# dalek-cryptography/zkp

Hardware: AMD Instinct MI355X
Metric: proofs/sec + batch-verifies/sec, CMZ13 10-attr credential, 1/2/4/8 MI355X (higher is better)
Workload: dtype u32x9 (29-bit limbs, u64 accumulate)

## Files before the change

include/zkp_mi355x.h:

```cpp
#ifndef ZKP_MI355X_H
#define ZKP_MI355X_H

#include <stddef.h>
#include <stdint.h>

#ifdef __cplusplus
extern "C" {
#endif

#define ZKP_OK 0
#define ZKP_ERR_HIP (-1)
#define ZKP_ERR_ARG (-2)
#define ZKP_ERR_NO_DEVICE (-3)
#define ZKP_ERR_OOM (-4)

#define ZKP_VARTIME 0
#define ZKP_CT 1

typedef struct zkp_ctx zkp_ctx;

int zkp_ctx_create(zkp_ctx** out, int device_id);
void zkp_ctx_destroy(zkp_ctx* ctx);
int zkp_ctx_set_stream(zkp_ctx* ctx, void* hip_stream);
int zkp_ctx_synchronize(zkp_ctx* ctx);
// ... 226 lines not shown
  ZKP_K_COUNT = 9
};
int zkp_ctx_last_timing(zkp_ctx* ctx, float* kernel_ms , float* total_ms);
int zkp_ctx_last_kernels(zkp_ctx* ctx, int kind, char* buf, size_t cap);
int zkp_ctx_set_profiling(zkp_ctx* ctx, int enabled);

#ifdef ZKP_BUILD_TEST_HOOKS
int zkp_debug_quad_selftest(zkp_ctx* ctx, uint32_t n, const uint8_t* pairs , uint8_t* out );
int zkp_debug_row_selftest(zkp_ctx* ctx, uint32_t n, const uint8_t* pairs , uint8_t* out );
int zkp_debug_wave_cycles(zkp_ctx* ctx, uint64_t* out, uint32_t cap);
int zkp_debug_sha512(zkp_ctx* ctx, uint64_t n, const uint8_t* msgs, const uint64_t* offsets , uint8_t* out );
int zkp_debug_last_schedule(zkp_ctx* ctx, char* buf, size_t cap);
int zkp_debug_ragged_blocks(const uint8_t* transcripts, uint32_t N, uint32_t* idx, uint32_t* blocks, uint32_t cap);
int zkp_debug_fill_workspace(zkp_ctx* ctx, size_t min_bytes, uint32_t word);
size_t zkp_debug_ws_bytes(zkp_ctx* ctx);
enum { ZKP_TESTOPT_DUMMY_LAUNCHES = 1001, ZKP_TESTOPT_GENERIC_CLASSIFIER = 1002, ZKP_TESTOPT_WAVE_CYCLES = 1003, ZKP_TESTOPT_PIP_MERGE = 1004, ZKP_TESTOPT_VOUCH_REDUCED = 1005 };
#endif

#ifdef __cplusplus
}
#endif
#endif
```

zkp_amd/csrc/comb_tables.h:

```cpp
#pragma once
#include "quad.h"
#include "stmt_pairs.h"

namespace zkp {

template <int TEETH>
struct comb_cfg {
  static_assert(TEETH == 4 || TEETH == 8 || TEETH == 16 || TEETH == 32, "teeth");
  static constexpr int BITS = 256 / TEETH;
  static constexpr int WINDOWS = BITS / 4;
  static constexpr int ENTRIES = 8 * TEETH + 1;
};
constexpr int comb_entries(int teeth) { return 8 * teeth + 1; }
constexpr int LADDER_ENTRIES = 8;

__device__ __forceinline__ void q_store_cached(dev_ext* dst, const qcached& c, int q) {
  uint32_t* w = reinterpret_cast<uint32_t*>(dst) + 9 * q;
#pragma unroll
  for (int i = 0; i < 9; ++i) w[i] = c.c.v[i];
}

__global__ void __launch_bounds__(256)
k_comb_slots(uint32_t n_points, const uint32_t* __restrict__ uses, uint32_t comb_min, uint32_t group_min, uint32_t max_tables,
             uint32_t* __restrict__ counter, uint32_t* __restrict__ slot_of, uint32_t* __restrict__ slot_pt, uint32_t* __restrict__ group_start,
// ... 274 lines not shown
        ge_cached_cmov(sel, n0, (uint32_t)(mag == 1));
        ge_cached_cmov(sel, n1, (uint32_t)(mag == 2));
#pragma unroll 1
        for (uint32_t h = 1; h < 4; ++h) {
          ge_cached c0, c1;
          load_comb_entry(c0, row + 2 * h + 0);
          load_comb_entry(c1, row + 2 * h + 1);
          ge_cached_cmov(sel, c0, (uint32_t)(mag == 2 * h + 1));
          ge_cached_cmov(sel, c1, (uint32_t)(mag == 2 * h + 2));
        }
        const dev_ext* next = (j + 1 < TEETH) ? row + 8 : tbl;
        load_comb_entry(n0, next + 0);
        load_comb_entry(n1, next + 1);
        if (fold && nidx == (int)SC_FOLD16_TOP_NIBBLE + 1) continue;
        ge_cached_cneg(sel, neg);
        if (w == cfg::WINDOWS - 1 && j == 0) ge_from_cached(acc, sel);
        else ge_add_cached(acc, acc, sel);
      }
    }
    if (fold) ge_cneg(acc, flip);
  } else {
#pragma unroll 1
    for (int w = cfg::WINDOWS - 1; w >= 0; --w) {
      if (w != cfg::WINDOWS - 1) {
        ge_double4(acc);
      }
#pragma unroll 1
      for (int j = 0; j < TEETH; ++j) {
        const int nidx = j * cfg::WINDOWS + w;
        const uint32_t nib = (ecol[256 * (nidx >> 3)] >> (4 * (nidx & 7))) & 15u;
        const uint32_t neg = (uint32_t)(nib < 8u);
        const uint32_t mag = neg ? 8u - nib : nib - 8u;
        ge_cached sel;
        comb_select<false>(sel, tbl + 8 * j, mag);
        ge_cached_cneg(sel, neg);
        if (w == cfg::WINDOWS - 1 && j == 0) ge_from_cached(acc, sel);
        else ge_add_cached(acc, acc, sel);
      }
    }
  }
  if (!no_carry) {
    ge_cached sel, c;
    ge_cached_identity(sel);
    load_comb_entry(c, tbl + 8 * TEETH);
    ge_cached_cmov(sel, c, top);
    ge_add_cached(acc, acc, sel);
  }
  store_ext(partial + t, acc);
}

__device__ __forceinline__ void ge_p3_dpp_from(ge_p3& r, const ge_p3& a, int ctrl_sel) {
  if (ctrl_sel == 0) { fe_dpp<ZKP_QP(1, 1, 3, 3)>(r.X, a.X); fe_dpp<ZKP_QP(1, 1, 3, 3)>(r.Y, a.Y); fe_dpp<ZKP_QP(1, 1, 3, 3)>(r.Z, a.Z); fe_dpp<ZKP_QP(1, 1, 3, 3)>(r.T, a.T); }
// ... 170 lines not shown
    const uint4* ent = lds + (size_t)row * 16 + col;
    uint32_t wd[36];
#pragma unroll
    for (int q = 0; q < 9; ++q) {
      const uint4 x = ent[q * 16];
      wd[4 * q + 0] = x.x; wd[4 * q + 1] = x.y; wd[4 * q + 2] = x.z; wd[4 * q + 3] = x.w;
    }
    fe_set(sel.YmX, wd); fe_set(sel.YpX, wd + 9); fe_set(sel.Z2, wd + 18); fe_set(sel.T2d, wd + 27);
  };
#pragma unroll 1
  for (int pass = 0; pass < 2; ++pass) {
    if (live && pass) {
      ge_double4(acc);
      ge_cached c;
      ge_to_cached(c, lo);
      ge_add_cached(acc, acc, c);
      ge_double4(acc);
    }
    uint32_t alo = pass ? dlo[1] : dlo[3], ahi = pass ? dhi[1] : dhi[3];
    uint32_t blo = pass ? dlo[0] : dlo[2], bhi = pass ? dhi[0] : dhi[2];
#pragma unroll 1
    for (int j = 0; j < 16; ++j) {
      asm volatile("s_waitcnt vmcnt(0)\n\ts_barrier" ::: "memory");
      ge_cached sel;
      uint32_t neg = 0;
      const bool first = pass == 0 && j == 0;
      if (live) {
        pick(alo, ahi, sel, neg);
        ge_cached_cneg(sel, neg);
        if (first) ge_from_cached(acc, sel);
        else ge_add_cached(acc, acc, sel);
        pick(blo, bhi, sel, neg);
      }
      lds_barrier();
      if (pass == 0 || j != 15) issue((uint32_t)((j + 1) & 15));
      if (live) {
        ge_cached_cneg(sel, neg);
        if (j == 0) ge_from_cached(lo, sel);
        else ge_add_cached(lo, lo, sel);
      }
    }
  }
  if (live) {
    ge_double4(acc);
    ge_cached c;
    ge_to_cached(c, lo);
// ... 103 lines not shown
      wd[4 * q + 0] = xbar_fetch(src, x.x); wd[4 * q + 1] = xbar_fetch(src, x.y);
      wd[4 * q + 2] = xbar_fetch(src, x.z); wd[4 * q + 3] = xbar_fetch(src, x.w);
    }
    const uint32_t m = 0u - nz, id = nz ^ 1u;
#pragma unroll
    for (int q = 0; q < 36; ++q) wd[q] &= m;
    wd[0] |= id; wd[9] |= id; wd[18] |= id << 1;
    fe_set(sel.YmX, wd); fe_set(sel.YpX, wd + 9); fe_set(sel.Z2, wd + 18); fe_set(sel.T2d, wd + 27);
  };
#pragma unroll 1
  for (int pass = 0; pass < 2; ++pass) {
    if (pass) {
      ge_double4(acc);
      ge_cached c;
      ge_to_cached(c, lo);
      ge_add_cached(acc, acc, c);
      ge_double4(acc);
    }
    uint32_t alo = pass ? dlo[1] : dlo[3], ahi = pass ? dhi[1] : dhi[3];
    uint32_t blo = pass ? dlo[0] : dlo[2], bhi = pass ? dhi[0] : dhi[2];
#pragma unroll 1
    for (int j = 0; j < 16; ++j) {
      asm volatile("s_waitcnt vmcnt(0)" ::: "memory");
      ge_cached sel;
      uint32_t neg = 0;
      const bool top_tooth = fold && pass == 0 && j == 15;
      if (!top_tooth) {
        pick(alo, ahi, sel, neg, false);
        ge_cached_cneg(sel, neg);
        if (pass == 0 && j == 0) ge_from_cached(acc, sel);
        else ge_add_cached(acc, acc, sel);
      }
      pick(blo, bhi, sel, neg, top_tooth);
      asm volatile("s_waitcnt lgkmcnt(0)" ::: "memory");
      if (pass == 0 || j != 15) issue((uint32_t)((j + 1) & 15));
      ge_cached_cneg(sel, neg);
      if (j == 0) ge_from_cached(lo, sel);
      else ge_add_cached(lo, lo, sel);
    }
  }
  ge_double4(acc);
  {
    ge_cached c;
    ge_to_cached(c, lo);
    ge_add_cached(acc, acc, c);
  }
// ... 89 lines not shown
#pragma unroll 1
  for (int j = 7; j >= 0; --j) {
    uint32_t cur = ecol[256 * j];
    int k = 0;
    if (folded && j == 7) { cur <<= 8; k = 2; }
#pragma unroll 1
    for (; k < 8; ++k) {
      ge_double4(acc);
      const uint32_t nib = cur >> 28;
      cur <<= 4;
      const uint32_t neg = (uint32_t)(nib < 8u);
      const uint32_t mag = neg ? 8u - nib : nib - 8u;
      ge_cached sel;
      ladder_select<CT>(sel, tbl, mag);
      ge_cached_cneg(sel, neg);
      ge_add_cached(acc, acc, sel);
    }
  }
  if (folded) ge_cneg(acc, flip);
  store_ext(partial + t, acc);
}

__global__ void __launch_bounds__(256, 2)
k_rider_tables(const uint32_t* __restrict__ n_slots, uint32_t max_tables, const uint32_t* __restrict__ slot_pt, const dev_affine* __restrict__ pts,
               dev_ext* __restrict__ comb) {
  __shared__ uint32_t stage[4][36][64];
  __shared__ uint32_t live[4][64];
  const uint32_t wave = threadIdx.x >> 6, lane = threadIdx.x & 63u;
  const uint32_t slot = blockIdx.x * blockDim.x + threadIdx.x, ns = min(*n_slots, max_tables);
  const uint32_t pi = slot < ns ? slot_pt[slot] : 0u;
  const bool have = slot < ns && (pi & STMT_ABSORBED);
// ... 109 lines not shown
```

zkp_amd/csrc/ge25519.h:

```cpp
#pragma once
#include "fe25519.h"
#include "fe_constants.h"

namespace zkp {

struct ge_p3 { fe X, Y, Z, T; };
struct ge_cached { fe YpX, YmX, Z2, T2d; };
struct ge_niels { fe ypx, ymx, xy2d; };

ZKP_HD void ge_identity(ge_p3& r) {
  fe_0(r.X);
  fe_1(r.Y);
  fe_1(r.Z);
  fe_0(r.T);
}
ZKP_HD void ge_cached_identity(ge_cached& r) {
  fe_1(r.YpX);
  fe_1(r.YmX);
  fe_0(r.Z2);
  r.Z2.v[0] = 2;
  FE_TRACK(fe_set_ub_exact(r.Z2));
  fe_0(r.T2d);
}
ZKP_HD void ge_niels_identity(ge_niels& r) {
// ... 12 lines not shown
  fe_carry(r.Z2, t);
  fe_from_const(d2, FE_D2);
  fe_mul(r.T2d, p.T, d2);
}

ZKP_HD void ge_affine_to_niels(ge_niels& r, const ge_p3& p) {
  fe t, d2;
  fe_add(t, p.Y, p.X);
  fe_carry(r.ypx, t);
  fe_sub(t, p.Y, p.X);
  fe_carry(r.ymx, t);
  fe_from_const(d2, FE_D2);
  fe_mul(r.xy2d, p.T, d2);
}

ZKP_HD void ge_add_cached(ge_p3& r, const ge_p3& p, const ge_cached& q) {
  fe a, b, c, d, e, f, g, h, t;
  fe_sub(t, p.Y, p.X);
  fe_mul(a, t, q.YmX);
  fe_add(t, p.Y, p.X);
  fe_mul(b, t, q.YpX);
  fe_mul(c, p.T, q.T2d);
  fe_mul(d, p.Z, q.Z2);
  fe_sub(e, b, a);
  fe_sub(t, d, c);
  fe_carry(f, t);
  fe_add(g, d, c);
  fe_add(h, b, a);
  fe_mul(r.X, e, f);
  fe_mul(r.Y, g, h);
  fe_mul(r.Z, f, g);
  fe_mul(r.T, e, h);
}

ZKP_HD void ge_sub_cached(ge_p3& r, const ge_p3& p, const ge_cached& q) {
  fe a, b, c, d, e, f, g, h, t;
  fe_sub(t, p.Y, p.X);
  fe_mul(a, t, q.YpX);
  fe_add(t, p.Y, p.X);
  fe_mul(b, t, q.YmX);
  fe_mul(c, p.T, q.T2d);
  fe_mul(d, p.Z, q.Z2);
  fe_sub(e, b, a);
  fe_add(t, d, c);
  fe_carry(f, t);
  fe_sub(g, d, c);
  fe_add(h, b, a);
  fe_mul(r.X, e, f);
  fe_mul(r.Y, g, h);
  fe_mul(r.Z, f, g);
  fe_mul(r.T, e, h);
}

ZKP_HD void ge_madd(ge_p3& r, const ge_p3& p, const ge_niels& q) {
  fe a, b, c, d, e, f, g, h, t;
  fe_sub(t, p.Y, p.X);
  fe_mul(a, t, q.ymx);
  fe_add(t, p.Y, p.X);
  fe_mul(b, t, q.ypx);
  fe_mul(c, p.T, q.xy2d);
  fe_add(d, p.Z, p.Z);
  fe_sub(e, b, a);
  fe_sub(t, d, c);
  fe_carry(f, t);
  fe_add(g, d, c);
  fe_add(h, b, a);
  fe_mul(r.X, e, f);
  fe_mul(r.Y, g, h);
  fe_mul(r.Z, f, g);
  fe_mul(r.T, e, h);
}

ZKP_HD void ge_msub(ge_p3& r, const ge_p3& p, const ge_niels& q) {
  fe a, b, c, d, e, f, g, h, t;
  fe_sub(t, p.Y, p.X);
  fe_mul(a, t, q.ypx);
  fe_add(t, p.Y, p.X);
  fe_mul(b, t, q.ymx);
  fe_mul(c, p.T, q.xy2d);
  fe_add(d, p.Z, p.Z);
  fe_sub(e, b, a);
  fe_add(t, d, c);
  fe_carry(f, t);
  fe_sub(t, d, c);
  fe_carry(g, t);
// ... 117 lines not shown
ZKP_HD void ge_cached_cmov(ge_cached& r, const ge_cached& q, uint32_t flag) {
  fe_cmov(r.YpX, q.YpX, flag);
  fe_cmov(r.YmX, q.YmX, flag);
  fe_cmov(r.Z2, q.Z2, flag);
  fe_cmov(r.T2d, q.T2d, flag);
}

ZKP_HD uint32_t fe_words_eq(const uint32_t w[8], const fe_words& c) {
  uint32_t x = 0;
#pragma unroll
  for (int i = 0; i < 8; ++i) x |= w[i] ^ c.w[i];
  return (uint32_t)(x == 0);
}

ZKP_HD uint32_t fe_invsqrt(fe& r, const fe& v) {
  fe t, v3, c;
  fe_sq(t, v);
  fe_mul(v3, t, v);
  fe_sq(t, v3);
  fe_mul(t, t, v);
  fe_pow22523(t, t);
  fe_mul(r, t, v3);
  fe_sq(t, r);
  fe_mul(t, t, v);
  uint32_t cw[8];
  fe_towords(cw, t);
  const uint32_t correct = fe_words_eq(cw, FE_W_ONE);
  const uint32_t flipped = fe_words_eq(cw, FE_W_MINUS_ONE);
  const uint32_t flipped_i = fe_words_eq(cw, FE_W_MINUS_SQRT_M1);
  fe_from_const(c, FE_SQRT_M1);
  fe_mul(t, r, c);
  fe_cmov(r, t, flipped | flipped_i);
  fe_abs(r, r);
  return correct | flipped;
}

ZKP_HD uint32_t fe_words_eq(const uint32_t a[8], const uint32_t b[8]) {
// ... 234 lines not shown
```

zkp_amd/csrc/point_mul.h:

```cpp
#pragma once
#include "comb_tables.h"

namespace zkp {

template <bool CT>
__device__ __forceinline__ void ladder16_point(ge_p3& acc, const uint32_t s[8], const ge_p3& P, uint4* tbl, uint32_t* ecol) {
  sc red;
#pragma unroll
  for (int j = 0; j < 8; ++j) red.v[j] = s[j];
  sc_reduce(red, red);
  uint32_t e[8];
  const uint32_t flip = sc_fold_recode16(e, red.v);
#pragma unroll
  for (int j = 0; j < 8; ++j) ecol[256 * j] = e[j];
  {
    ge_p3 m2, m3, m4, m;
    ge_cached c1, c;
    ge_to_cached(c1, P);
    ladder_store_entry(tbl, 0, c1);
    ge_double<true>(m2, P);
    ge_to_cached(c, m2); ladder_store_entry(tbl, 1, c);
    ge_add_cached(m3, m2, c1);
    ge_to_cached(c, m3); ladder_store_entry(tbl, 2, c);
    ge_double<true>(m4, m2);
// ... 15 lines not shown
#pragma unroll 1
  for (int j = 7; j >= 0; --j) {
    uint32_t cur = ecol[256 * j];
    int k = 0;
    if (j == 7) { cur <<= 8; k = 2; }
#pragma unroll 1
    for (; k < 8; ++k) {
      ge_double4(acc);
      const uint32_t nib = cur >> 28;
      cur <<= 4;
      const uint32_t neg = (uint32_t)(nib < 8u);
      const uint32_t mag = neg ? 8u - nib : nib - 8u;
      ge_cached sel;
      ladder_select<CT>(sel, tbl, mag);
      ge_cached_cneg(sel, neg);
      ge_add_cached(acc, acc, sel);
    }
  }
  ge_cneg(acc, flip);
}

}
```

zkp_amd/csrc/zkp_kernels.hip:

```cpp
#include <hip/hip_runtime.h>
#include <sys/syscall.h>
#include <unistd.h>
#include <cctype>
#include <cstdio>
#include <cstring>
#include <algorithm>
#include <atomic>
#include <functional>
#include <map>
#include <memory>
#include <mutex>
#include <set>
#include <string>
#include <vector>
#include "../../include/zkp_mi355x.h"
#include "dev_layout.h"

using namespace zkp;

__device__ __forceinline__ uint32_t sel8(const uint32_t w[8], int j) {
  uint32_t r = w[0];
#pragma unroll
  for (int i = 1; i < 8; ++i) r = (j == i) ? w[i] : r;
  return r;
// ... 832 lines not shown
  q_load_ext(t, rin, q);
  q_add(run, run, t, q);
#pragma unroll 1
  for (int k = 0; k < shift; ++k) q_double(U, U, q);
  if (level > 0) {
    const dev_ext* ain = A_in + (size_t)w * in_stride + (size_t)m * j;
#pragma unroll 1
    for (int i = 0; i < m; ++i) {
      q_load_ext(t, ain + i, q);
      q_add(U, U, t, q);
    }
  }
  q_store_ext(A_out + (size_t)w * out_stride + j, U, q);
  if (R_out) q_store_ext(R_out + (size_t)w * out_stride + j, run, q);
}
__global__ void __launch_bounds__(256, 2)
k_pip_reduce_lvl(uint32_t n_out, uint32_t total, uint32_t in_stride, uint32_t out_stride, int level, int m, int shift,
                 const dev_ext* __restrict__ A_in, const dev_ext* __restrict__ R_in,
                 dev_ext* __restrict__ A_out, dev_ext* __restrict__ R_out) {
  const uint32_t gt = blockIdx.x * blockDim.x + threadIdx.x;
  const uint32_t g = gt >> 2;
  const int q = (int)(gt & 3u);
  if (g >= total) return;
  pip_reduce_quad(g, q, n_out, in_stride, out_stride, level, m, shift, A_in, R_in, A_out, R_out);
}

__global__ void __launch_bounds__(256)
k_pip_combine(int W1, int C, uint32_t in_stride, int level, int m, int shift, const dev_ext* __restrict__ A_in, const dev_ext* __restrict__ R_in,
              dev_ext* __restrict__ T_all, const uint32_t* __restrict__ invalid, uint8_t* __restrict__ out_point, uint32_t* __restrict__ status,
              uint32_t shared_flags ) {
  const uint32_t b = blockIdx.x;
  dev_ext* T = T_all + (size_t)b * W1;
  const uint32_t g = threadIdx.x >> 2;
  const int q = (int)(threadIdx.x & 3u);
  if (g < (uint32_t)W1) pip_reduce_quad(b * (uint32_t)W1 + g, q, 1u, in_stride, 1u, level, m, shift, A_in, R_in, T_all, nullptr);
  __syncthreads();
  __shared__ uint32_t Tl[64 * 36];
  if (g < (uint32_t)W1) {
    qpt t;
// ... 692 lines not shown
  int fuse_tables_transcript = -1;
  int tables_lane = -1;
  int comb_split = -1;
  int grouped_comb = -1;
  int ladder_interleave = -1;
  static constexpr uint32_t kInterleaveLadderBlocks = 256;
  bool each_straus = true;
  uint32_t each_straus_lanes = 0;
  uint32_t each_straus_wins = 0;
  int ct_lookup = 0;
#ifdef ZKP_BUILD_TEST_HOOKS
  uint64_t* wave_cycles = nullptr;
  static constexpr uint32_t kWaveCyclesCap = 1u << 20;
  enum { SCH_BATCH_ENCODE, SCH_ENC_GROUPS, SCH_OPT_PIP, SCH_PIP_C, SCH_PIP_PART, SCH_STATUS_SHARED, SCH_LAT_SPLIT, SCH_GROUPED, SCH_COMB_MIN,
         SCH_LADDER_INTERLEAVE, SCH_RIDERS, SCH_STRAUS_LANES, SCH_STRAUS_WINS, SCH_TR_LANES, SCH_TR_STEPS, SCH_FUSE_TT, SCH_TERMS_SPLIT,
         SCH_RAGGED_CLASSES, SCH_RAGGED_COMPILED, SCH_RAGGED_BASE, SCH_FUSED_PLANS, SCH_PIP_MERGE, SCH_PIP_BUCKETS, SCH_NO_CARRY, SCH_SIGN_FOLD, SCH_COUNT };
  int64_t sched[SCH_COUNT] = {-1, -1, -1, -1, -1, -1, -1, -1, -1, -1, -1, -1, -1, -1, -1, -1, -1, -1, -1, -1, -1, -1, -1, -1, -1};
  int debug_pip_merge = 0;
  bool debug_vouch_reduced = false;
#endif
  static constexpr size_t kGroupedCombTerms = 400000;
  static constexpr size_t kSplitCombTerms = 8192;
  bool dev_overlap = false;
  bool dev_latency = false;
  bool rider_tables = true;
  bool joint_ladder = true;
  bool tr_steps = true;
  int tr_lanes = -1;
  static constexpr size_t kWideCallTerms = 250000, kWideCallProofs = 8192;
  static constexpr size_t kVeryWideCallProofs = 65536;
  uint32_t ct_comb_min(bool throughput, size_t n_terms) const {
    return ct_single_use_tables < 0 ? (throughput && n_terms >= kWideCallTerms ? 2u : 1u) : (ct_single_use_tables ? 1u : 2u);
  }
// ... 448 lines not shown
  if (!shared_flags) HIP_TRY(hipMemsetAsync(invalid, 0, (size_t)K * 4, c->stream));
  prof_note(c, ZKP_K_DECODE, "k_pip_prepare<" + std::to_string(C) + ">");
  if (phases == 2) hipLaunchKernelGGL((k_pip_prepare<C, 2>), dim3((n + 255) / 256, K), dim3(256), 0, c->stream, n, seg, d_scalars, d_points, niels, digits, invalid);
  else hipLaunchKernelGGL((k_pip_prepare<C, 3>), dim3((n + 255) / 256, K), dim3(256), 0, c->stream, n, seg, d_scalars, d_points, niels, digits, invalid);
  prof_mark(c, ZKP_K_DECODE);
  hipLaunchKernelGGL(k_pip_tile_hist<C>, dim3(tiles, (unsigned)WK), dim3(sort_cfg<C>::THREADS), 0, c->stream, n, digits, tilehist);
  hipLaunchKernelGGL(k_pip_tile_total, grid1(nb, 256), dim3(256), 0, c->stream, cfg::B1, tiles, (uint32_t)nb, tilehist, hist);
  hipLaunchKernelGGL(k_pip_scan, dim3((unsigned)WK), dim3(256), 0, c->stream, cfg::B1, L, hist, start, cursor, vstart);
  hipLaunchKernelGGL(k_pip_tile_base, grid1(nb, 256), dim3(256), 0, c->stream, cfg::B1, tiles, (uint32_t)nb, start, tilehist);
  hipLaunchKernelGGL(k_pip_tile_scatter<C>, dim3(tiles, (unsigned)WK), dim3(sort_cfg<C>::THREADS), 0, c->stream, n, digits, tilehist, sorted);
  prof_mark(c, ZKP_K_SORT);
  hipLaunchKernelGGL(k_pip_vmap, grid1(nb, 256), dim3(256), 0, c->stream, cfg::B1, (uint32_t)nb, (uint32_t)vmax, vstart, vmap);
  hipLaunchKernelGGL(k_pip_bucket_part, dim3((unsigned)((vmax + 255) / 256), (unsigned)WK), dim3(256), 0, c->stream, n, (uint32_t)cfg::W1, cfg::B1, L, (uint32_t)vmax,
                     start, hist, vstart, vmap, sorted, niels, parts);
  constexpr size_t MERGE_LANE_MIN_BUCKETS = (size_t)1 << 19;
#ifdef ZKP_BUILD_TEST_HOOKS
  const bool lane_merge = c->debug_pip_merge ? c->debug_pip_merge == 2 : nb >= MERGE_LANE_MIN_BUCKETS;
#else
  const bool lane_merge = nb >= MERGE_LANE_MIN_BUCKETS;
#endif
  ZKP_SCHED(c, PIP_MERGE, lane_merge ? 1 : 0);
  ZKP_SCHED(c, PIP_BUCKETS, nb);
  if (lane_merge) hipLaunchKernelGGL(k_pip_bucket_merge<true>, grid1(nb, 256), dim3(256), 0, c->stream, cfg::B1, (uint32_t)nb, (uint32_t)vmax, vstart, parts, buckets);
  else hipLaunchKernelGGL(k_pip_bucket_merge<false>, grid1(nb * 4, 256), dim3(256), 0, c->stream, cfg::B1, (uint32_t)nb, (uint32_t)vmax, vstart, parts, buckets);
  prof_mark(c, ZKP_K_BUCKET);
  const dev_ext* Ain = nullptr;
  const dev_ext* Rin = buckets;
  uint32_t in_stride = cfg::B1, n_in = cfg::B;
  size_t lvl_off = 0;
  int level = 0;
  int shift = 0;
  static_assert(cfg::W1 <= 64, "k_pip_combine runs the last tree level with one quad per window in one 256-lane block");
  while (n_in > 1) {
    int lg = 0;
    while ((1u << lg) < n_in) ++lg;
    const int mbits = (level == 0 && lg % 3) ? lg % 3 : 3;
    const uint32_t m = 1u << mbits, n_out = n_in >> mbits;
    dev_ext* Aout = lvlA + lvl_off;
    dev_ext* Rout = lvlR + lvl_off;
    const uint32_t total = (uint32_t)WK * n_out;
    if (n_out == 1) {
      hipLaunchKernelGGL(k_pip_combine, dim3(K), dim3(256), 0, c->stream, cfg::W1, C, in_stride, level, (int)m, shift, Ain, Rin, Aout, invalid, d_out, d_status, shared_flags ? 1u : 0u);
      break;
    }
    hipLaunchKernelGGL(k_pip_reduce_lvl, grid1((size_t)total * 4, 256), dim3(256), 0, c->stream, n_out, total, in_stride, n_out, level, (int)m, shift,
                       Ain, Rin, Aout, Rout);
    Ain = Aout;
    Rin = Rout;
    in_stride = n_out;
    n_in = n_out;
    lvl_off += total;
    shift += mbits;
    ++level;
  }
  prof_mark(c, ZKP_K_COMBINE);
  HIP_TRY(hipGetLastError());
  return ZKP_OK;
}

int pick_c(uint64_t n) {
  if (n < (1u << 12)) return 7;
  if (n < (1u << 13)) return 10;
  if (n < (1u << 21)) return 11;
  return 16;
}
constexpr uint64_t kSmallOptional = 192;

terms_cfg host_terms_cfg(const zkp_ctx* c, uint32_t n_terms, const uint32_t* pidx, const uint8_t* points, uint32_t n_points, uint32_t comb_min) {
  std::vector<uint32_t> uses(n_points, 0);
// ... 479 lines not shown

int zkp_ctx_set_stream(zkp_ctx* c, void* s) {
  if (!c) return fail(ZKP_ERR_ARG, "ctx is NULL");
  c->stream = s ? static_cast<hipStream_t>(s) : c->own_stream;
  return ZKP_OK;
}
int zkp_ctx_set_option(zkp_ctx* c, int option, uint64_t value) {
  if (!c) return fail(ZKP_ERR_ARG, "ctx is NULL");
  switch (option) {
    case ZKP_OPT_BATCH_ENCODE_MIN: c->batch_encode_min = value; c->batch_encode_user = true; return ZKP_OK;
    case ZKP_OPT_CT_SINGLE_USE_TABLES: c->ct_single_use_tables = value == ~0ull ? -1 : (value ? 1 : 0); return ZKP_OK;
    case ZKP_OPT_DEV_OVERLAP: c->dev_overlap = value != 0 && value != ~0ull; c->dev_latency = value == 2; return ZKP_OK;
#ifdef ZKP_BUILD_TEST_HOOKS
    case ZKP_TESTOPT_GENERIC_CLASSIFIER: c->stmt_classify = value == 0; return ZKP_OK;
    case ZKP_TESTOPT_PIP_MERGE: c->debug_pip_merge = value <= 2 ? (int)value : 0; return ZKP_OK;
    case ZKP_TESTOPT_VOUCH_REDUCED: c->debug_vouch_reduced = value != 0; return ZKP_OK;
    case ZKP_TESTOPT_DUMMY_LAUNCHES: c->debug_dummy_launches = (int)std::min<uint64_t>(value, 1000); return ZKP_OK;
    case ZKP_TESTOPT_WAVE_CYCLES: {
      HIP_TRY(hipSetDevice(c->device));
      HIP_TRY(hipStreamSynchronize(c->stream));
      uint64_t* p = nullptr;
      uint32_t cap = 0;
      if (value) {
        if (!c->wave_cycles) HIP_TRY(hipMalloc(&c->wave_cycles, sizeof(uint64_t) * zkp_ctx::kWaveCyclesCap));
        HIP_TRY(hipMemset(c->wave_cycles, 0, sizeof(uint64_t) * zkp_ctx::kWaveCyclesCap));
        p = c->wave_cycles;
        cap = zkp_ctx::kWaveCyclesCap;
      }
      HIP_TRY(hipMemcpyToSymbol(HIP_SYMBOL(g_wave_cycles), &p, sizeof(p)));
      HIP_TRY(hipMemcpyToSymbol(HIP_SYMBOL(g_wave_cycles_cap), &cap, sizeof(cap)));
// ... 374 lines not shown
    if (pidx) HIP_TRY(hipMemcpyAsync(base + o_pidx, pidx, (size_t)n_terms * 4, hipMemcpyHostToDevice, c->stream));
    HIP_TRY(hipMemcpyAsync(base + o_pts, points, (size_t)n_points * 32, hipMemcpyHostToDevice, c->stream));
  }
  prof_begin(c);
  if (!pidx && n_terms) hipLaunchKernelGGL(k_iota, grid1(n_terms, 256), dim3(256), 0, c->stream, n_terms, reinterpret_cast<uint32_t*>(base + o_pidx));
  rc = launch_msm_segments(c, n_msm, reinterpret_cast<uint32_t*>(base + o_off), reinterpret_cast<uint8_t*>(base + o_sc), reinterpret_cast<uint32_t*>(base + o_pidx),
                           reinterpret_cast<uint8_t*>(base + o_pts), n_points, n_terms, flags, k, w, reinterpret_cast<uint8_t*>(base + o_out),
                           reinterpret_cast<uint8_t*>(base + o_st));
  if (rc) return rc;
  HIP_TRY(hipMemcpyAsync(out, base + o_out, (size_t)n_msm * 32, hipMemcpyDeviceToHost, c->stream));
  HIP_TRY(hipMemcpyAsync(status, base + o_st, (size_t)n_msm, hipMemcpyDeviceToHost, c->stream));
  HIP_TRY(hipStreamSynchronize(c->stream));
  return ZKP_OK;
}

static int msm_optional_impl(zkp_ctx* c, uint64_t n, const uint8_t* d_scalars, const uint8_t* d_points,
                             uint8_t* d_out, uint32_t* d_status, size_t reserved, uint32_t* shared_flags = nullptr, int phases = 3) {
  ZKP_SCHED(c, OPT_PIP, n > kSmallOptional);
  if (n <= kSmallOptional) {
    if (shared_flags) return fail(ZKP_ERR_ARG, "internal: shared flags with a small MSM");
    carve cv;
    cv.off = reserved;
    const size_t o_pidx = cv.take((size_t)(n + 1) * 4);
    const size_t o_off = cv.take(256);
    const size_t inner = cv.off;
    int rc = ensure_ws(c, inner + terms_path_ws((uint32_t)n, (uint32_t)n, 1));
    if (rc) return rc;
    char* base = static_cast<char*>(c->ws);
    uint32_t* pidx = reinterpret_cast<uint32_t*>(base + o_pidx);
    uint32_t* off = reinterpret_cast<uint32_t*>(base + o_off);
    hipLaunchKernelGGL(k_iota_single_msm, grid1(n + 1, 256), dim3(256), 0, c->stream, (uint32_t)n, pidx, off);
    return msm_terms_path(c, 1, off, d_scalars, pidx, d_points, (uint32_t)n, (uint32_t)n, ZKP_VARTIME, d_out, nullptr, d_status, inner);
  }
  if (n > 0x7fffffffull) return fail(ZKP_ERR_ARG, "n too large (max 2^31-1 terms per call)");
  const int cbits = pick_c(n);
  size_t need = 0;
  switch (cbits) {
    case 7: need = pip_ws<7>(n); break;
    case 10: need = pip_ws<10>(n); break;
    case 11: need = pip_ws<11>(n); break;
    default: need = pip_ws<16>(n); break;
  }
  int rc = ensure_ws(c, reserved + need);
  if (rc) return rc;
  switch (cbits) {
    case 7: return pip_run<7>(c, (uint32_t)n, d_scalars, d_points, d_out, d_status, reserved, shared_flags, pip_seg(), phases);
    case 10: return pip_run<10>(c, (uint32_t)n, d_scalars, d_points, d_out, d_status, reserved, shared_flags, pip_seg(), phases);
    case 11: return pip_run<11>(c, (uint32_t)n, d_scalars, d_points, d_out, d_status, reserved, shared_flags, pip_seg(), phases);
    default: return pip_run<16>(c, (uint32_t)n, d_scalars, d_points, d_out, d_status, reserved, shared_flags, pip_seg(), phases);
  }
// ... 13 lines not shown
int zkp_msm_optional(zkp_ctx* c, uint64_t n, const uint8_t* scalars, const uint8_t* points, uint8_t out_point[32], int* status) {
  if (!c) return fail(ZKP_ERR_ARG, "ctx is NULL");
  if (!out_point || !status) return fail(ZKP_ERR_ARG, "NULL output pointer");
  if (n && (!scalars || !points)) return fail(ZKP_ERR_ARG, "NULL input pointer");
  HIP_TRY(hipSetDevice(c->device));
  carve cv;
  const size_t o_sc = cv.take((size_t)n * 32 + 32);
  const size_t o_pts = cv.take((size_t)n * 32 + 32);
  const size_t o_out = cv.take(32);
  const size_t o_st = cv.take(4);
  const size_t reserved = cv.off;
  size_t need = 0;
  if (n <= kSmallOptional) {
    need = 1024 + (n + 1) * 4 + terms_path_ws((uint32_t)n, (uint32_t)n, 1);
  } else {
    switch (pick_c(n)) {
      case 7: need = pip_ws<7>(n); break;
      case 10: need = pip_ws<10>(n); break;
      case 11: need = pip_ws<11>(n); break;
        default: need = pip_ws<16>(n); break;
    }
  }
  int rc = ensure_ws(c, reserved + need);
  if (rc) return rc;
  char* base = static_cast<char*>(c->ws);
  if (n) {
    HIP_TRY(hipMemcpyAsync(base + o_sc, scalars, (size_t)n * 32, hipMemcpyHostToDevice, c->stream));
    HIP_TRY(hipMemcpyAsync(base + o_pts, points, (size_t)n * 32, hipMemcpyHostToDevice, c->stream));
  }
  prof_begin(c);
  rc = msm_optional_impl(c, n, reinterpret_cast<uint8_t*>(base + o_sc), reinterpret_cast<uint8_t*>(base + o_pts),
// ... 492 lines not shown
  HIP_TRY(hipMemcpyAsync(base + o_ts, ts, 208 * (size_t)N, hipMemcpyHostToDevice, c->stream));
  prof_begin(c);
  rc = launch_strobe_challenge(c, N, base + o_ts, lab, len, base + o_out);
  if (rc) return rc;
  HIP_TRY(hipMemcpyAsync(ts, base + o_ts, 208 * (size_t)N, hipMemcpyDeviceToHost, c->stream));
  if (len) HIP_TRY(hipMemcpyAsync(out, base + o_out, (size_t)N * len, hipMemcpyDeviceToHost, c->stream));
  HIP_TRY(hipStreamSynchronize(c->stream));
  return ZKP_OK;
}

#ifdef ZKP_BUILD_TEST_HOOKS
int zkp_debug_last_schedule(zkp_ctx* c, char* buf, size_t cap) {
  if (!c || !buf || !cap) return fail(ZKP_ERR_ARG, "bad argument");
  static const char* const names[zkp_ctx::SCH_COUNT] = {"batch_encode", "enc_groups", "opt_pip", "pip_c", "pip_part", "status_shared", "lat_split", "grouped", "comb_min",
                                                        "ladder_interleave", "riders", "straus_lanes", "straus_wins", "tr_lanes", "tr_steps", "fuse_tt", "terms_split",
                                                        "ragged_classes", "ragged_compiled", "ragged_base", "fused_plans", "pip_merge", "pip_buckets", "no_carry", "sign_fold"};
  std::string s;
  for (int i = 0; i < zkp_ctx::SCH_COUNT; ++i)
    if (c->sched[i] >= 0) s += (s.empty() ? "" : " ") + std::string(names[i]) + "=" + std::to_string(c->sched[i]);
  const size_t n = std::min(s.size(), cap - 1);
  memcpy(buf, s.data(), n);
  buf[n] = 0;
  return (int)s.size();
}

int zkp_debug_sha512(zkp_ctx* c, uint64_t n, const uint8_t* msgs, const uint64_t* offsets, uint8_t* out) {
  return hash_from_bytes_host(c, n, msgs, offsets, out, HASH_DIGEST);
}
#endif

#ifdef ZKP_BUILD_TEST_HOOKS
// ... 96 lines not shown
```

zkp_amd/engine.py:

```python
from __future__ import annotations

import ctypes
import os
from typing import Optional, Sequence, Tuple

import numpy as np

from . import cabi

_HERE = os.path.dirname(os.path.abspath(__file__))
LIB_PATH = os.path.join(_HERE, "libzkp_mi355x.so")
TESTHOOKS_LIB_PATH = os.path.join(_HERE, "libzkp_mi355x_testhooks.so")
ZKP_TESTOPT_DUMMY_LAUNCHES, ZKP_TESTOPT_GENERIC_CLASSIFIER, ZKP_TESTOPT_WAVE_CYCLES, ZKP_TESTOPT_PIP_MERGE, ZKP_TESTOPT_VOUCH_REDUCED = 1001, 1002, 1003, 1004, 1005
ZKP_OPT_CT_LOOKUP, ZKP_OPT_EACH_STRAUS, ZKP_OPT_LADDER_INTERLEAVE = 9, 10, 11
ZKP_OPT_CT_MASKED_SCANS = ZKP_OPT_CT_LOOKUP
ZKP_CT_LOOKUP_XBAR, ZKP_CT_LOOKUP_SCAN, ZKP_CT_LOOKUP_LDS = 0, 1, 2
ZKP_OPT_WS_LIMIT_BYTES, ZKP_OPT_JOB_DEFER_D2H, ZKP_OPT_SYNC_SCHEDULE, ZKP_OPT_TRANSCRIPT_STEPS, ZKP_OPT_COMB_SPLIT, ZKP_OPT_JOINT_LADDER = 12, 13, 14, 15, 16, 17

ZKP_VARTIME = 0
ZKP_CT = 1
ZKP_PT_ADD, ZKP_PT_SUB = 0, 1
ZKP_DLOG_FOUND, ZKP_DLOG_INVALID, ZKP_DLOG_NOT_FOUND = 0, 1, 2
ZKP_OPT_BATCH_ENCODE_MIN = 1
(ZKP_OPT_COMB_TEETH, ZKP_OPT_CT_SINGLE_USE_TABLES, ZKP_OPT_TRANSCRIPT_LANES, ZKP_OPT_DEV_OVERLAP, ZKP_OPT_GROUPED_COMB, ZKP_OPT_TABLES_LANE,
 ZKP_OPT_FUSE_TABLES_TRANSCRIPT) = 2, 3, 4, 5, 6, 7, 8
K_NAMES = ("decode", "terms", "reduce", "sort", "bucket", "combine", "transcript", "scalars", "tables")

EXPORTS = tuple(cabi.signatures("zkp_mi355x.h"))
# ... 665 lines not shown
```

Measured before the change: 4.606 million.

## Skip dead T products before doublings, add per-lane PIP reduce, simplify invsqrt

Point additions whose result feeds straight into a doubling now skip the final T = e*h field multiply, since doubling does not read T. This saves one fe_mul per such addition across the comb, ladder and PIP paths. A new one-thread-per-output PIP tree reduction kernel replaces the quad-cooperative version when there are many outputs. fe_invsqrt now calls pow22523 on v directly, dropping several multiplies. Test hooks are added to force the tree mode and the window size. The risks are that the garbage T might be read on some path, and that the invsqrt rewrite might change the math.

```diff
diff --git a/include/zkp_mi355x.h b/include/zkp_mi355x.h
--- a/include/zkp_mi355x.h
+++ b/include/zkp_mi355x.h
@@ -264,7 +264,7 @@
 int zkp_debug_ragged_blocks(const uint8_t* transcripts, uint32_t N, uint32_t* idx, uint32_t* blocks, uint32_t cap);
 int zkp_debug_fill_workspace(zkp_ctx* ctx, size_t min_bytes, uint32_t word);
 size_t zkp_debug_ws_bytes(zkp_ctx* ctx);
-enum { ZKP_TESTOPT_DUMMY_LAUNCHES = 1001, ZKP_TESTOPT_GENERIC_CLASSIFIER = 1002, ZKP_TESTOPT_WAVE_CYCLES = 1003, ZKP_TESTOPT_PIP_MERGE = 1004, ZKP_TESTOPT_VOUCH_REDUCED = 1005 };
+enum { ZKP_TESTOPT_DUMMY_LAUNCHES = 1001, ZKP_TESTOPT_GENERIC_CLASSIFIER = 1002, ZKP_TESTOPT_WAVE_CYCLES = 1003, ZKP_TESTOPT_PIP_MERGE = 1004, ZKP_TESTOPT_VOUCH_REDUCED = 1005, ZKP_TESTOPT_PIP_TREE = 1006, ZKP_TESTOPT_PIP_C = 1007 };
 #endif
 
 #ifdef __cplusplus
diff --git a/zkp_amd/csrc/comb_tables.h b/zkp_amd/csrc/comb_tables.h
--- a/zkp_amd/csrc/comb_tables.h
+++ b/zkp_amd/csrc/comb_tables.h
@@ -312,8 +312,9 @@
         load_comb_entry(n1, next + 1);
         if (fold && nidx == (int)SC_FOLD16_TOP_NIBBLE + 1) continue;
         ge_cached_cneg(sel, neg);
+        const bool into_doubling = w != 0 && j == ((fold && w == cfg::WINDOWS - 1) ? TEETH - 2 : TEETH - 1);
         if (w == cfg::WINDOWS - 1 && j == 0) ge_from_cached(acc, sel);
-        else ge_add_cached(acc, acc, sel);
+        else ge_add_cached(acc, acc, sel, !into_doubling);
       }
     }
     if (fold) ge_cneg(acc, flip);
@@ -333,7 +334,7 @@
         comb_select<false>(sel, tbl + 8 * j, mag);
         ge_cached_cneg(sel, neg);
         if (w == cfg::WINDOWS - 1 && j == 0) ge_from_cached(acc, sel);
-        else ge_add_cached(acc, acc, sel);
+        else ge_add_cached(acc, acc, sel, w == 0 || j != TEETH - 1);
       }
     }
   }
@@ -534,7 +535,7 @@
       ge_double4(acc);
       ge_cached c;
       ge_to_cached(c, lo);
-      ge_add_cached(acc, acc, c);
+      ge_add_cached<false>(acc, acc, c);
       ge_double4(acc);
     }
     uint32_t alo = pass ? dlo[1] : dlo[3], ahi = pass ? dhi[1] : dhi[3];
@@ -549,7 +550,7 @@
         pick(alo, ahi, sel, neg);
         ge_cached_cneg(sel, neg);
         if (first) ge_from_cached(acc, sel);
-        else ge_add_cached(acc, acc, sel);
+        else ge_add_cached(acc, acc, sel, j != 15);
         pick(blo, bhi, sel, neg);
       }
       lds_barrier();
@@ -683,7 +684,7 @@
       ge_double4(acc);
       ge_cached c;
       ge_to_cached(c, lo);
-      ge_add_cached(acc, acc, c);
+      ge_add_cached<false>(acc, acc, c);
       ge_double4(acc);
     }
     uint32_t alo = pass ? dlo[1] : dlo[3], ahi = pass ? dhi[1] : dhi[3];
@@ -698,7 +699,7 @@
         pick(alo, ahi, sel, neg, false);
         ge_cached_cneg(sel, neg);
         if (pass == 0 && j == 0) ge_from_cached(acc, sel);
-        else ge_add_cached(acc, acc, sel);
+        else ge_add_cached(acc, acc, sel, j != ((fold && pass == 0) ? 14 : 15));
       }
       pick(blo, bhi, sel, neg, top_tooth);
       asm volatile("s_waitcnt lgkmcnt(0)" ::: "memory");
@@ -818,7 +819,7 @@
       ge_cached sel;
       ladder_select<CT>(sel, tbl, mag);
       ge_cached_cneg(sel, neg);
-      ge_add_cached(acc, acc, sel);
+      ge_add_cached(acc, acc, sel, j == 0 && k == 7);
     }
   }
   if (folded) ge_cneg(acc, flip);
diff --git a/zkp_amd/csrc/ge25519.h b/zkp_amd/csrc/ge25519.h
--- a/zkp_amd/csrc/ge25519.h
+++ b/zkp_amd/csrc/ge25519.h
@@ -50,7 +50,13 @@
   fe_mul(r.xy2d, p.T, d2);
 }
 
-ZKP_HD void ge_add_cached(ge_p3& r, const ge_p3& p, const ge_cached& q) {
+ZKP_HD void ge_skip_t(ge_p3& r) {
+  FE_TRACK(for (int i = 0; i < 9; ++i) { r.T.v[i] = 0x2aaaaaaau; r.T.ub[i] = 1ull << 40; });
+  (void)r;
+}
+
+template <bool WITH_T = true>
+ZKP_HD void ge_add_cached(ge_p3& r, const ge_p3& p, const ge_cached& q, bool with_t = true) {
   fe a, b, c, d, e, f, g, h, t;
   fe_sub(t, p.Y, p.X);
   fe_mul(a, t, q.YmX);
@@ -66,10 +72,12 @@
   fe_mul(r.X, e, f);
   fe_mul(r.Y, g, h);
   fe_mul(r.Z, f, g);
-  fe_mul(r.T, e, h);
-}
-
-ZKP_HD void ge_sub_cached(ge_p3& r, const ge_p3& p, const ge_cached& q) {
+  if (WITH_T && with_t) fe_mul(r.T, e, h);
+  else ge_skip_t(r);
+}
+
+template <bool WITH_T = true>
+ZKP_HD void ge_sub_cached(ge_p3& r, const ge_p3& p, const ge_cached& q, bool with_t = true) {
   fe a, b, c, d, e, f, g, h, t;
   fe_sub(t, p.Y, p.X);
   fe_mul(a, t, q.YpX);
@@ -85,10 +93,12 @@
   fe_mul(r.X, e, f);
   fe_mul(r.Y, g, h);
   fe_mul(r.Z, f, g);
-  fe_mul(r.T, e, h);
-}
-
-ZKP_HD void ge_madd(ge_p3& r, const ge_p3& p, const ge_niels& q) {
+  if (WITH_T && with_t) fe_mul(r.T, e, h);
+  else ge_skip_t(r);
+}
+
+template <bool WITH_T = true>
+ZKP_HD void ge_madd(ge_p3& r, const ge_p3& p, const ge_niels& q, bool with_t = true) {
   fe a, b, c, d, e, f, g, h, t;
   fe_sub(t, p.Y, p.X);
   fe_mul(a, t, q.ymx);
@@ -104,7 +114,8 @@
   fe_mul(r.X, e, f);
   fe_mul(r.Y, g, h);
   fe_mul(r.Z, f, g);
-  fe_mul(r.T, e, h);
+  if (WITH_T && with_t) fe_mul(r.T, e, h);
+  else ge_skip_t(r);
 }
 
 ZKP_HD void ge_msub(ge_p3& r, const ge_p3& p, const ge_niels& q) {
@@ -252,13 +263,8 @@
 }
 
 ZKP_HD uint32_t fe_invsqrt(fe& r, const fe& v) {
-  fe t, v3, c;
-  fe_sq(t, v);
-  fe_mul(v3, t, v);
-  fe_sq(t, v3);
-  fe_mul(t, t, v);
-  fe_pow22523(t, t);
-  fe_mul(r, t, v3);
+  fe t, c;
+  fe_pow22523(r, v);
   fe_sq(t, r);
   fe_mul(t, t, v);
   uint32_t cw[8];
diff --git a/zkp_amd/csrc/point_mul.h b/zkp_amd/csrc/point_mul.h
--- a/zkp_amd/csrc/point_mul.h
+++ b/zkp_amd/csrc/point_mul.h
@@ -53,7 +53,7 @@
       ge_cached sel;
       ladder_select<CT>(sel, tbl, mag);
       ge_cached_cneg(sel, neg);
-      ge_add_cached(acc, acc, sel);
+      ge_add_cached(acc, acc, sel, j == 0 && k == 7);
     }
   }
   ge_cneg(acc, flip);
diff --git a/zkp_amd/csrc/zkp_kernels.hip b/zkp_amd/csrc/zkp_kernels.hip
--- a/zkp_amd/csrc/zkp_kernels.hip
+++ b/zkp_amd/csrc/zkp_kernels.hip
@@ -870,15 +870,58 @@
   q_store_ext(A_out + (size_t)w * out_stride + j, U, q);
   if (R_out) q_store_ext(R_out + (size_t)w * out_stride + j, run, q);
 }
+__device__ __forceinline__ void pip_reduce_lane(uint32_t g, uint32_t n_out, uint32_t in_stride, uint32_t out_stride, int level, int m, int shift,
+                                                const dev_ext* __restrict__ A_in, const dev_ext* __restrict__ R_in,
+                                                dev_ext* __restrict__ A_out, dev_ext* __restrict__ R_out) {
+  const uint32_t w = g / n_out, j = g - w * n_out;
+  const dev_ext* rin = R_in + (size_t)w * in_stride + (size_t)m * j;
+  const int first = (level == 0 && j == n_out - 1) ? m : m - 1;
+  ge_p3 run, U, nx;
+  ge_cached c;
+  load_ext(run, rin + first);
+  U = run;
+  load_ext(nx, rin + first - 1);
+#pragma unroll 1
+  for (int i = first - 1; i >= 1; --i) {
+    ge_to_cached(c, nx);
+    load_ext(nx, rin + i - 1);
+    ge_add_cached(run, run, c);
+    ge_to_cached(c, run);
+    ge_add_cached(U, U, c, i != 1 || shift == 0);
+  }
+  ge_to_cached(c, nx);
+  const dev_ext* ain = level > 0 ? A_in + (size_t)w * in_stride + (size_t)m * j : nullptr;
+  if (level > 0) load_ext(nx, ain);
+  ge_add_cached(run, run, c);
+#pragma unroll 1
+  for (int k = 1; k < shift; ++k) ge_double<false>(U, U);
+  if (shift > 0) ge_double<true>(U, U);
+  if (level > 0) {
+#pragma unroll 1
+    for (int i = 0; i < m; ++i) {
+      ge_to_cached(c, nx);
+      if (i + 1 < m) load_ext(nx, ain + i + 1);
+      ge_add_cached(U, U, c);
+    }
+  }
+  store_ext(A_out + (size_t)w * out_stride + j, U);
+  store_ext(R_out + (size_t)w * out_stride + j, run);
+}
+template <bool LANE>
 __global__ void __launch_bounds__(256, 2)
 k_pip_reduce_lvl(uint32_t n_out, uint32_t total, uint32_t in_stride, uint32_t out_stride, int level, int m, int shift,
                  const dev_ext* __restrict__ A_in, const dev_ext* __restrict__ R_in,
                  dev_ext* __restrict__ A_out, dev_ext* __restrict__ R_out) {
   const uint32_t gt = blockIdx.x * blockDim.x + threadIdx.x;
-  const uint32_t g = gt >> 2;
-  const int q = (int)(gt & 3u);
-  if (g >= total) return;
-  pip_reduce_quad(g, q, n_out, in_stride, out_stride, level, m, shift, A_in, R_in, A_out, R_out);
+  if constexpr (LANE) {
+    if (gt >= total) return;
+    pip_reduce_lane(gt, n_out, in_stride, out_stride, level, m, shift, A_in, R_in, A_out, R_out);
+  } else {
+    const uint32_t g = gt >> 2;
+    const int q = (int)(gt & 3u);
+    if (g >= total) return;
+    pip_reduce_quad(g, q, n_out, in_stride, out_stride, level, m, shift, A_in, R_in, A_out, R_out);
+  }
 }
 
 __global__ void __launch_bounds__(256)
@@ -1601,9 +1644,11 @@
   static constexpr uint32_t kWaveCyclesCap = 1u << 20;
   enum { SCH_BATCH_ENCODE, SCH_ENC_GROUPS, SCH_OPT_PIP, SCH_PIP_C, SCH_PIP_PART, SCH_STATUS_SHARED, SCH_LAT_SPLIT, SCH_GROUPED, SCH_COMB_MIN,
          SCH_LADDER_INTERLEAVE, SCH_RIDERS, SCH_STRAUS_LANES, SCH_STRAUS_WINS, SCH_TR_LANES, SCH_TR_STEPS, SCH_FUSE_TT, SCH_TERMS_SPLIT,
-         SCH_RAGGED_CLASSES, SCH_RAGGED_COMPILED, SCH_RAGGED_BASE, SCH_FUSED_PLANS, SCH_PIP_MERGE, SCH_PIP_BUCKETS, SCH_NO_CARRY, SCH_SIGN_FOLD, SCH_COUNT };
-  int64_t sched[SCH_COUNT] = {-1, -1, -1, -1, -1, -1, -1, -1, -1, -1, -1, -1, -1, -1, -1, -1, -1, -1, -1, -1, -1, -1, -1, -1, -1};
+         SCH_RAGGED_CLASSES, SCH_RAGGED_COMPILED, SCH_RAGGED_BASE, SCH_FUSED_PLANS, SCH_PIP_MERGE, SCH_PIP_BUCKETS, SCH_NO_CARRY, SCH_SIGN_FOLD, SCH_PIP_TREE, SCH_COUNT };
+  int64_t sched[SCH_COUNT] = {-1, -1, -1, -1, -1, -1, -1, -1, -1, -1, -1, -1, -1, -1, -1, -1, -1, -1, -1, -1, -1, -1, -1, -1, -1, -1};
   int debug_pip_merge = 0;
+  int debug_pip_tree = 0;
+  int debug_pip_c = 0;
   bool debug_vouch_reduced = false;
 #endif
   static constexpr size_t kGroupedCombTerms = 400000;
@@ -2082,6 +2127,7 @@
   hipLaunchKernelGGL(k_pip_bucket_part, dim3((unsigned)((vmax + 255) / 256), (unsigned)WK), dim3(256), 0, c->stream, n, (uint32_t)cfg::W1, cfg::B1, L, (uint32_t)vmax,
                      start, hist, vstart, vmap, sorted, niels, parts);
   constexpr size_t MERGE_LANE_MIN_BUCKETS = (size_t)1 << 19;
+  constexpr uint32_t REDUCE_LANE_MIN_OUTPUTS = 1u << 16;
 #ifdef ZKP_BUILD_TEST_HOOKS
   const bool lane_merge = c->debug_pip_merge ? c->debug_pip_merge == 2 : nb >= MERGE_LANE_MIN_BUCKETS;
 #else
@@ -2098,6 +2144,7 @@
   size_t lvl_off = 0;
   int level = 0;
   int shift = 0;
+  int tree_lanes = 0;
   static_assert(cfg::W1 <= 64, "k_pip_combine runs the last tree level with one quad per window in one 256-lane block");
   while (n_in > 1) {
     int lg = 0;
@@ -2111,8 +2158,16 @@
       hipLaunchKernelGGL(k_pip_combine, dim3(K), dim3(256), 0, c->stream, cfg::W1, C, in_stride, level, (int)m, shift, Ain, Rin, Aout, invalid, d_out, d_status, shared_flags ? 1u : 0u);
       break;
     }
-    hipLaunchKernelGGL(k_pip_reduce_lvl, grid1((size_t)total * 4, 256), dim3(256), 0, c->stream, n_out, total, in_stride, n_out, level, (int)m, shift,
-                       Ain, Rin, Aout, Rout);
+#ifdef ZKP_BUILD_TEST_HOOKS
+    const bool lane_lvl = c->debug_pip_tree ? c->debug_pip_tree == 2 : total >= REDUCE_LANE_MIN_OUTPUTS;
+#else
+    const bool lane_lvl = total >= REDUCE_LANE_MIN_OUTPUTS;
+#endif
+    if (lane_lvl) tree_lanes |= 1 << level;
+    if (lane_lvl) hipLaunchKernelGGL(k_pip_reduce_lvl<true>, grid1((size_t)total, 256), dim3(256), 0, c->stream, n_out, total, in_stride, n_out, level, (int)m, shift,
+                                     Ain, Rin, Aout, Rout);
+    else hipLaunchKernelGGL(k_pip_reduce_lvl<false>, grid1((size_t)total * 4, 256), dim3(256), 0, c->stream, n_out, total, in_stride, n_out, level, (int)m, shift,
+                            Ain, Rin, Aout, Rout);
     Ain = Aout;
     Rin = Rout;
     in_stride = n_out;
@@ -2121,6 +2176,7 @@
     shift += mbits;
     ++level;
   }
+  ZKP_SCHED(c, PIP_TREE, tree_lanes);
   prof_mark(c, ZKP_K_COMBINE);
   HIP_TRY(hipGetLastError());
   return ZKP_OK;
@@ -2630,6 +2686,8 @@
 #ifdef ZKP_BUILD_TEST_HOOKS
     case ZKP_TESTOPT_GENERIC_CLASSIFIER: c->stmt_classify = value == 0; return ZKP_OK;
     case ZKP_TESTOPT_PIP_MERGE: c->debug_pip_merge = value <= 2 ? (int)value : 0; return ZKP_OK;
+    case ZKP_TESTOPT_PIP_TREE: c->debug_pip_tree = value <= 2 ? (int)value : 0; return ZKP_OK;
+    case ZKP_TESTOPT_PIP_C: c->debug_pip_c = (value == 7 || value == 10 || value == 11 || value == 16) ? (int)value : 0; return ZKP_OK;
     case ZKP_TESTOPT_VOUCH_REDUCED: c->debug_vouch_reduced = value != 0; return ZKP_OK;
     case ZKP_TESTOPT_DUMMY_LAUNCHES: c->debug_dummy_launches = (int)std::min<uint64_t>(value, 1000); return ZKP_OK;
     case ZKP_TESTOPT_WAVE_CYCLES: {
@@ -3034,6 +3092,14 @@
   return ZKP_OK;
 }
 
+static int optional_c(const zkp_ctx* c, uint64_t n) {
+#ifdef ZKP_BUILD_TEST_HOOKS
+  if (c->debug_pip_c) return c->debug_pip_c;
+#endif
+  (void)c;
+  return pick_c(n);
+}
+
 static int msm_optional_impl(zkp_ctx* c, uint64_t n, const uint8_t* d_scalars, const uint8_t* d_points,
                              uint8_t* d_out, uint32_t* d_status, size_t reserved, uint32_t* shared_flags = nullptr, int phases = 3) {
   ZKP_SCHED(c, OPT_PIP, n > kSmallOptional);
@@ -3053,7 +3119,7 @@
     return msm_terms_path(c, 1, off, d_scalars, pidx, d_points, (uint32_t)n, (uint32_t)n, ZKP_VARTIME, d_out, nullptr, d_status, inner);
   }
   if (n > 0x7fffffffull) return fail(ZKP_ERR_ARG, "n too large (max 2^31-1 terms per call)");
-  const int cbits = pick_c(n);
+  const int cbits = optional_c(c, n);
   size_t need = 0;
   switch (cbits) {
     case 7: need = pip_ws<7>(n); break;
@@ -3097,7 +3163,7 @@
   if (n <= kSmallOptional) {
     need = 1024 + (n + 1) * 4 + terms_path_ws((uint32_t)n, (uint32_t)n, 1);
   } else {
-    switch (pick_c(n)) {
+    switch (optional_c(c, n)) {
       case 7: need = pip_ws<7>(n); break;
       case 10: need = pip_ws<10>(n); break;
       case 11: need = pip_ws<11>(n); break;
@@ -3620,7 +3686,7 @@
   if (!c || !buf || !cap) return fail(ZKP_ERR_ARG, "bad argument");
   static const char* const names[zkp_ctx::SCH_COUNT] = {"batch_encode", "enc_groups", "opt_pip", "pip_c", "pip_part", "status_shared", "lat_split", "grouped", "comb_min",
                                                         "ladder_interleave", "riders", "straus_lanes", "straus_wins", "tr_lanes", "tr_steps", "fuse_tt", "terms_split",
-                                                        "ragged_classes", "ragged_compiled", "ragged_base", "fused_plans", "pip_merge", "pip_buckets", "no_carry", "sign_fold"};
+                                                        "ragged_classes", "ragged_compiled", "ragged_base", "fused_plans", "pip_merge", "pip_buckets", "no_carry", "sign_fold", "pip_tree"};
   std::string s;
   for (int i = 0; i < zkp_ctx::SCH_COUNT; ++i)
     if (c->sched[i] >= 0) s += (s.empty() ? "" : " ") + std::string(names[i]) + "=" + std::to_string(c->sched[i]);
diff --git a/zkp_amd/engine.py b/zkp_amd/engine.py
--- a/zkp_amd/engine.py
+++ b/zkp_amd/engine.py
@@ -11,7 +11,7 @@
 _HERE = os.path.dirname(os.path.abspath(__file__))
 LIB_PATH = os.path.join(_HERE, "libzkp_mi355x.so")
 TESTHOOKS_LIB_PATH = os.path.join(_HERE, "libzkp_mi355x_testhooks.so")
-ZKP_TESTOPT_DUMMY_LAUNCHES, ZKP_TESTOPT_GENERIC_CLASSIFIER, ZKP_TESTOPT_WAVE_CYCLES, ZKP_TESTOPT_PIP_MERGE, ZKP_TESTOPT_VOUCH_REDUCED = 1001, 1002, 1003, 1004, 1005
+ZKP_TESTOPT_DUMMY_LAUNCHES, ZKP_TESTOPT_GENERIC_CLASSIFIER, ZKP_TESTOPT_WAVE_CYCLES, ZKP_TESTOPT_PIP_MERGE, ZKP_TESTOPT_VOUCH_REDUCED, ZKP_TESTOPT_PIP_TREE, ZKP_TESTOPT_PIP_C = 1001, 1002, 1003, 1004, 1005, 1006, 1007
 ZKP_OPT_CT_LOOKUP, ZKP_OPT_EACH_STRAUS, ZKP_OPT_LADDER_INTERLEAVE = 9, 10, 11
 ZKP_OPT_CT_MASKED_SCANS = ZKP_OPT_CT_LOOKUP
 ZKP_CT_LOOKUP_XBAR, ZKP_CT_LOOKUP_SCAN, ZKP_CT_LOOKUP_LDS = 0, 1, 2
```

Measured after the change: 4.575 million. No clear change (-0.7%).
